# Ai00-X/ai00_server

Hardware: AMD Instinct MI355X
Metric: decode tokens/sec (whole job) (higher is better)
Workload: dtype u8->f16/f32acc; 1 GPU; RWKV-v6-3b int8 decode, batch=32/GPU, greedy, state+tokens resident in HBM; quant=int8, batch_per_gpu=32, parallelism=replicas x1 (no collective)

## Files before the change

ai00_server_amd/build.py:

```python
from __future__ import annotations

import os
import subprocess
import sys

HERE = os.path.dirname(os.path.abspath(__file__))
CSRC = os.path.join(HERE, "csrc")
LIB = os.path.join(HERE, "librwkv_hip.so")
SOURCES = ["rwkv_kernels.hip", "rwkv_engine.cpp", "tokenizer.cpp"]
DEPS = SOURCES + ["rwkv_kernels.h", "gemm_plan.h", "graph_cache.h", "gen_stop.h", "safetensors.hpp", "rwkv_abi.map", os.path.join("..", "..", "include", "rwkv_abi.h"),
               os.path.join("..", "..", "include", "rwkv_runtime.hpp"), os.path.join("..", "..", "include", "rwkv_scheduler.hpp"),
               os.path.join("..", "..", "include", "rwkv_router.hpp"),
               os.path.join("..", "..", "harness", "decode_loop.cpp"), os.path.join("..", "..", "harness", "serve_loop.cpp"),
               os.path.join("..", "..", "harness", "router_loop.cpp")]


def _hipcc() -> str:
    for c in (os.environ.get("HIPCC"), "/opt/rocm/bin/hipcc", "hipcc"):
        if c and (os.path.isabs(c) and os.path.exists(c) or not os.path.isabs(c)):
            return c
    return "hipcc"


STAMP = os.path.join(HERE, ".build_stamp")


def _sources_digest() -> str:
    import hashlib
    h = hashlib.sha256()
    for d in sorted(DEPS):
        with open(os.path.join(CSRC, d), "rb") as f:
            h.update(d.encode())
            h.update(f.read())
# ... 72 lines not shown
```

ai00_server_amd/csrc/gemm_plan.h:

```cpp
#pragma once
#include "rwkv_kernels.h"
#include <algorithm>

namespace rwkv {

struct Opd {
    _Float16 *hi = nullptr, *lo = nullptr;
    int ld = 0;
};

struct ProbSpec {
    const DMat *W = nullptr;
    Opd x;
    int xoff = 0;
    int act = ACT_NONE, post = POST_NONE;
    const float *bias = nullptr, *m0 = nullptr, *m1 = nullptr;
    int ldm = 0;
    float *out = nullptr;
    int ldo = 0;
    bool partial = false;
    Opd oh;
};

struct ProbShape {
    int rows, K, fmt;
    bool partial;
    bool kcopies;
    bool smallk;
};
inline ProbShape shape_of(const ProbSpec &s) {
    return {s.W->rows, s.W->K, s.W->fmt, s.partial, s.post != POST_MIX && s.act == ACT_NONE && !s.bias && !s.oh.hi,
            s.xoff == 0 && s.out && !s.oh.hi && s.post == POST_NONE};
}

inline void fill_prob(GemmProb &g, const ProbSpec &s, long pstride) {
    g.W = s.W->data; g.S = s.W->scales; g.fmt = s.W->fmt; g.rows = s.W->rows; g.K = s.W->K;
    g.xhi = s.x.hi + (s.xoff >> 5) * 512; g.xlo = s.x.lo ? s.x.lo + (s.xoff >> 5) * 512 : nullptr; g.ldx = s.x.ld;
    g.act = s.act; g.post = s.post; g.bias = s.bias; g.m0 = s.m0; g.m1 = s.m1; g.ldm = s.ldm;
    g.out_f32 = s.out; g.ldo = s.ldo; g.partial_stride = pstride;
    g.out_hi = s.oh.hi; g.out_lo = s.oh.lo; g.ldh = s.oh.ld;
}

inline void gemm_variant(int T, bool hilo, int &NT, int &KSW) {
    KSW = 8;
// ... 208 lines not shown
```

ai00_server_amd/csrc/rwkv_engine.cpp:

```cpp
#include <hip/hip_runtime.h>

#include <algorithm>
#include <cmath>
#include <cstdio>
#include <cstdlib>
#include <cstring>
#include <map>
#include <memory>
#include <mutex>
#include <numeric>
#include <optional>
#include <stdexcept>
#include <string>
#include <vector>

#include "../../include/rwkv_abi.h"
#include "gemm_plan.h"
#include "graph_cache.h"
#include "safetensors.hpp"

using namespace rwkv;

static thread_local std::string g_err;
struct RwkvError : std::runtime_error {
// ... 235 lines not shown
    float *d_score_out = nullptr, *h_score_out = nullptr, *d_soft_score = nullptr, *h_soft_score = nullptr;
    Opd opA[6], opM, opY, opK, opO, opL[4];
    long pstride = 0;
    int *d_meta = nullptr, *h_meta = nullptr;
    MetaView dm;
    static constexpr int META_RING = 4;
    hipEvent_t meta_ev[META_RING] = {nullptr, nullptr, nullptr, nullptr};
    int meta_next = 0;
    int *h_tok = nullptr, *dv_tok = nullptr;
    StepPlan last_plan;
    std::vector<size_t> last_ntok;
    std::vector<int> last_opt;
    uint64_t plan_counter = 0, uploaded_id = 0;
    size_t meta_cap = 0;
    int *d_tok_feedback = nullptr, *d_hist = nullptr, *d_amax_i = nullptr;
    int *d_adj_row = nullptr, *d_adj_tok = nullptr;
    float *d_adj_val = nullptr;
    unsigned char *d_allow = nullptr, *h_allow = nullptr;
    int *d_allow_row = nullptr;
    SampStage samp{};
    static constexpr size_t ADJ_CAP = 1 << 16;
    float *d_amax_v = nullptr;
    size_t hist_cap = 0;

    bool profiling = false;
    float prof_ms[RWKV_PROFILE_FAMILIES] = {0};
    int prof_n[RWKV_PROFILE_FAMILIES] = {0};
    hipEvent_t ev0 = nullptr, ev1 = nullptr;

    GraphCacheOf<uint64_t> graphs{64, {}};
    std::optional<GraphCacheOf<int>> greedy_graphs;
    static constexpr int GEN_RING_STEPS = 1024;
    std::vector<GenSlot> gen_host;
    std::vector<char> gen_armed;
    std::vector<std::vector<uint32_t>> gen_prompt;
    std::vector<size_t> gen_ppos;
    std::vector<float *> gen_shadow;
    GenSlot *d_gen = nullptr;
    GenStop *d_gen_stop = nullptr;
    std::vector<char> gen_has_stops;
    unsigned *d_tok_off = nullptr;
    unsigned char *d_tok_bytes = nullptr;
    int n_tok = 0;
    void gen_set_token_bytes(const uint8_t *bytes, const int32_t *lens, size_t n);
    void gen_set_stops(int slot, const rwkv_gen_stops &s);
    size_t gen_stop_tail(int slot, uint8_t *out, size_t cap);
// ... 92 lines not shown
        } else {
            f();
        }
    }
    void prof_collect() {
        HIP_CHECK(hipStreamSynchronize(s_main));
        for (size_t i = 0; i < prof_fam.size(); ++i) {
            float ms = 0;
            HIP_CHECK(hipEventElapsedTime(&ms, prof_ev[2 * i], prof_ev[2 * i + 1]));
            prof_ms[prof_fam[i]] += ms;
            prof_n[prof_fam[i]] += 1;
        }
        prof_fam.clear();
    }

    void load(const rwkv_load_desc &d);
    int gemm(std::vector<ProbSpec> &ps, int T, int fam, const ShiftCommit *commit = nullptr, int cls = CLS_NONE);
    void log_gemm(const std::vector<ProbSpec> &ps, int T, int fam, const char *kind, int variant, int grid, int ksplit, int threads);
    void log_row(const char *kernel, int T, long grid, double bytes);
    int step_max_rows = 0;
    float *lnp_xx_att = nullptr;
    void plan_step(const rwkv_slot_input *in, StepPlan &pl);
    void upload_plan(const StepPlan &pl);
    void run_layers(int T, int n_seq, int n_out, const int *d_token, bool dense);
    void infer(const rwkv_slot_input *in, rwkv_slot_output *out);
    void run_plan(const StepPlan &pl);
    void infer_sample(const rwkv_slot_input *in, const rwkv_sample_params *sp, uint32_t *out_tokens, float *out_probs,
                      uint8_t *emitted, size_t *n_consumed);
    void infer_score(const rwkv_slot_input *in, const uint32_t *const *targets, float *const *out_logp, size_t *n_consumed);
    std::vector<rwkv_slot_input> one_token_each(const std::vector<int> &slots, const uint32_t *tokens) const {
        static const uint32_t none = 0;
        std::vector<rwkv_slot_input> in((size_t)max_batch, rwkv_slot_input{nullptr, 0, RWKV_OPTION_LAST, 0});
        for (size_t i = 0; i < slots.size(); ++i) in[(size_t)slots[i]] = rwkv_slot_input{tokens ? tokens + i : &none, 1, RWKV_OPTION_LAST, 0};
        return in;
    }
};

static bool lora_scope(const std::string &name) {
    if (name.compare(0, 7, "blocks.") != 0) return false;
    size_t i = 7;
    while (i < name.size() && name[i] >= '0' && name[i] <= '9') ++i;
    return i > 7 && i + 1 < name.size() && name[i] == '.';
}

static bool is_quant_target(int version, const std::string &suffix) {
    static const char *att56[] = {"att.receptance.weight", "att.key.weight", "att.value.weight", "att.output.weight", "att.gate.weight"};
    static const char *att7[] = {"att.receptance.weight", "att.key.weight", "att.value.weight", "att.output.weight"};
// ... 370 lines not shown
    for (auto &ev : meta_ev) HIP_CHECK(hipEventCreateWithFlags(&ev, hipEventDisableTiming));
    h_tok = hostalloc<int>((size_t)max_batch, hipHostMallocMapped | hipHostMallocCoherent);
    HIP_CHECK(hipHostGetDevicePointer((void **)&dv_tok, h_tok, 0));
    d_tok_feedback = dalloc<int>(chunk);
    soft_rows_cap = (size_t)std::max(1, max_batch);
    soft_in = dalloc<float>(soft_rows_cap * V);
    soft_out = dalloc<float>(soft_rows_cap * V);
    soft_host = hostalloc<float>(soft_rows_cap * V);
    d_score_tgt = dalloc<unsigned>(chunk); d_score_out = dalloc<float>(chunk);
    h_score_tgt = hostalloc<unsigned>(chunk); h_score_out = hostalloc<float>(chunk);
    d_soft_tgt = dalloc<unsigned>(soft_rows_cap); d_soft_score = dalloc<float>(soft_rows_cap);
    h_soft_tgt = hostalloc<unsigned>(soft_rows_cap); h_soft_score = hostalloc<float>(soft_rows_cap);
    d_adj_row = dalloc<int>(ADJ_CAP); d_adj_tok = dalloc<int>(ADJ_CAP); d_adj_val = dalloc<float>(ADJ_CAP);
    d_allow = dalloc<unsigned char>((size_t)max_batch * V); d_allow_row = dalloc<int>(max_batch);
    h_allow = hostalloc<unsigned char>((size_t)max_batch * V + (size_t)max_batch * 4 + 16);
    const size_t o_adj = (size_t)chunk * sizeof(SampleRow), o_out = o_adj + ADJ_CAP * 12, samp_bytes = o_out + (size_t)chunk * 8;
    unsigned char *h_samp = hostalloc<unsigned char>(samp_bytes);
    unsigned char *dv_samp = nullptr;
    HIP_CHECK(hipHostGetDevicePointer((void **)&dv_samp, h_samp, 0));
    int *adj = (int *)(h_samp + o_adj), *out = (int *)(h_samp + o_out), *dv_out = (int *)(dv_samp + o_out);
    samp = SampStage{(SampleRow *)h_samp, adj, adj + ADJ_CAP, (float *)(adj + 2 * ADJ_CAP), out, (float *)(out + chunk),
                     (const SampleRow *)dv_samp, dv_out, (float *)(dv_out + chunk)};
    greedy_graphs.emplace((size_t)max_batch, GraphExecDeleter{});
    d_amax_v = dalloc<float>((size_t)chunk * 32);
    d_amax_i = dalloc<int>((size_t)chunk * 32);
    HIP_CHECK(hipDeviceSynchronize());
}

int rwkv_engine::gemm(std::vector<ProbSpec> &ps, int T, int fam, const ShiftCommit *commit, int cls) {
    const bool hilo = wide(cls);
    if (hilo) for (auto &sp : ps) if (!sp.x.lo) throw RwkvError(RWKV_ERR_INVALID, "gemm: a hi + lo launch needs the lo part of every operand");
    if (ps.empty() || ps.size() > GEMM_MAXP) throw RwkvError(RWKV_ERR_INVALID, "gemm: bad problem count");
    const int n = (int)ps.size();
    ProbShape sh[GEMM_MAXP];
    for (int i = 0; i < n; ++i) sh[i] = shape_of(ps[i]);
    GemmLaunch Lh;
    const GemmPlan pl = plan_gemm(Lh, sh, n, T, hilo, commit && commit->src, kn);
    if (!pl.ksplit) throw RwkvError(RWKV_ERR_UNSUPPORTED, "cannot split inner dimension");
    for (int i = 0; i < n; ++i) fill_prob(Lh.p[i], ps[i], pstride);
    if (pl.path == GEMM_DECODE && commit) Lh.commit = *commit;
    log_gemm(ps, T, fam, kGemmPathNames[pl.path], pl.variant, pl.grid, pl.ksplit, pl.threads);
    if (pl.path == GEMM_SMALLK) launch(fam, [&] { launch_smallk(Lh, hilo, s_main); });
    else if (pl.path == GEMM_TILE) launch(fam, [&] { launch_gemm_tile(Lh, pl.variant, hilo, s_main); });
    else launch(fam, [&] { launch_gemm(Lh, hilo, s_main); });
    return pl.ksplit;
}

void rwkv_engine::log_row(const char *kernel, int T, long grid, double bytes) {
    if (!launch_log || cur_layer > 1) return;
    std::fprintf(launch_log, "{\"kind\": \"row\", \"kernel\": \"%s\", \"T\": %d, \"grid\": %ld, \"bytes\": %.0f}\n", kernel, T, grid, bytes);
    std::fflush(launch_log);
}
void rwkv_engine::log_gemm(const std::vector<ProbSpec> &ps, int T, int fam, const char *kind, int variant, int grid, int ksplit, int threads) {
    if (!launch_log || (cur_layer > 1 && fam != FAM_HEAD)) return;
    uint64_t bytes = 0;
    double flops = 0;
    long rows = 0;
    std::string names;
    for (auto &sp : ps) {
        bytes += sp.W->bytes;
        rows += sp.W->rows;
        flops += 2.0 * T * (double)sp.W->rows * sp.W->K;
        for (auto &kv : mats)
// ... 71 lines not shown
    last_ntok.assign(B, 0);
    last_opt.assign(B, 0);
    for (int b = 0; b < B; ++b) { last_ntok[b] = in[b].n_tokens; last_opt[b] = in[b].option; }
}

void rwkv_engine::upload_plan(const StepPlan &pl) {
    const int slot = meta_next;
    meta_next = (meta_next + 1) % META_RING;
    HIP_CHECK(hipEventSynchronize(meta_ev[slot]));
    const MetaView h(h_meta + (size_t)slot * meta_cap, chunk, max_batch);
    std::memcpy(h.token, pl.token.data(), pl.T * 4);
    std::memcpy(h.slot, pl.slot.data(), pl.T * 4);
    std::memcpy(h.prev, pl.prev.data(), pl.T * 4);
    std::memcpy(h.last, pl.last.data(), pl.T * 4);
    std::memcpy(h.out_rows, pl.out_rows.data(), pl.n_out * 4);
    std::memcpy(h.seq_slot, pl.seq_slot.data(), pl.n_seq * 4);
    std::memcpy(h.seq_begin, pl.seq_begin.data(), pl.n_seq * 4);
    std::memcpy(h.seq_len, pl.seq_len.data(), pl.n_seq * 4);
    HIP_CHECK(hipMemcpyAsync(d_meta, h.token, meta_cap * 4, hipMemcpyHostToDevice, s_main));
    HIP_CHECK(hipEventRecord(meta_ev[slot], s_main));
    uploaded_id = pl.id;
}

void rwkv_engine::run_layers(int T, int n_seq, int n_out, const int *d_token, bool dense) {
    const int C = info.num_emb, V = info.num_vocab, H = info.num_head, L = info.num_layer;
    const RowMeta rm{d_token, dm.slot, dm.prev, dm.last, dense ? 1 : 0};

    float *cur = xA, *oth = xB;
    int np = 0;
    {
        EmbedArgs e{emb, ln0w, ln0b, d_token, cur, C, V};
        launch(FAM_ROW, [&] { launch_embed(e, T, s_main); });
    }
    for (int l = 0; l < L; ++l) {
        const LayerW &w = layers[l];
        cur_layer = l;
        LnShiftArgs a{};
        a.x_in = cur; a.x_out = oth; a.P = P; a.np = np; a.pstride = pstride;
        a.lnw = w.ln1w; a.lnb = w.ln1b;
        a.sx = sxa + (long)l * C; a.sx_slot_stride = sx_slot_stride;
        a.rm = rm; a.C = C; a.ldh = C;
        std::vector<ProbSpec> ps;
        auto prob = [&](const DMat *W, const Opd &x, int act, float *out, int ldo) {
            ProbSpec s; s.W = W; s.x = x; s.act = act; s.out = out; s.ldo = ldo; return s;
        };
        auto as = [&](const Opd &o, int cls) { Opd r = o; if (!wide(cls)) r.lo = nullptr; return r; };
        const Opd aA[6] = {as(opA[0], CLS_ATT), as(opA[1], CLS_ATT), as(opA[2], CLS_ATT), as(opA[3], CLS_ATT), as(opA[4], CLS_ATT), as(opA[5], CLS_ATT)};
        const Opd aL[4] = {as(opL[0], CLS_LORA2), as(opL[1], CLS_LORA2), as(opL[2], CLS_LORA2), as(opL[3], CLS_LORA2)};
        const Opd aF[2] = {as(opA[0], CLS_FFN1), as(opA[1], CLS_FFN1)};
        const Opd aY = as(opY, CLS_WO), aK = as(opK, CLS_FV), aZ = as(opA[0], CLS_NONE), aM = as(opM, CLS_NONE);
        auto ln_pro = [&](const LnShiftArgs &r, float *xx_pub) {
            LnProArgs lp{};
            lp.x_in = r.x_in; lp.x_out = r.x_out; lp.P = r.P; lp.np = r.np; lp.pstride = r.pstride;
// ... 118 lines not shown
            ProbSpec s = prob(w.Fk, aF[0], ACT_RELU2, nullptr, 0);
            s.oh = aK;
            ps = {s};
            if (info.version != 7) { ProbSpec r = prob(w.Fr, aF[1], ACT_SIGMOID, frr, C); ps.push_back(r); }
            { launch(FAM_ROW, [&] { launch_ln_shift(f, T, s_main); }); log_ln(f); }
            gemm(ps, T, FAM_GEMM, nullptr, CLS_FFN1);
            std::swap(cur, oth);
        }
        {
            ProbSpec s = prob(w.Fv, aK, ACT_NONE, P, C);
            s.partial = true;
            if (info.version != 7) { s.post = POST_MUL; s.m0 = frr; s.ldm = C; }
            ps = {s};
            np = gemm(ps, T, FAM_GEMM, nullptr, CLS_FV);
        }
    }
    if (n_out > 0) {
        Opd aO = opO;
        if (!wide(CLS_HEAD)) aO.lo = nullptr;
        LnOutArgs o{cur, P, np, pstride, lnow, lnob, dense ? nullptr : dm.out_rows, aO.hi, aO.lo, C, C};
        launch(FAM_ROW, [&] { launch_ln_out(o, n_out, s_main); });
        std::vector<ProbSpec> ps(1);
        ps[0].W = head; ps[0].x = aO; ps[0].out = logits; ps[0].ldo = V;
        gemm(ps, n_out, FAM_HEAD, nullptr, CLS_HEAD);
    } else if (np > 0) {
    }
}

void rwkv_engine::run_plan(const StepPlan &pl) {
    if (pl.dense) std::memcpy(h_tok, pl.token.data(), (size_t)pl.T * 4);
    if (!pl.dense || pl.id != uploaded_id) upload_plan(pl);
    const int *tok_ptr = pl.dense ? dv_tok : dm.token;
    step_max_rows = pl.max_rows();
    const bool short_rows = step_max_rows <= 8;
    const uint64_t key = ((uint64_t)pl.dense << 63) | ((uint64_t)short_rows << 62) | ((uint64_t)pl.T << 40) | ((uint64_t)pl.n_seq << 20) | (uint64_t)pl.n_out;
    auto enqueue = [&] { run_layers(pl.T, pl.n_seq, pl.n_out, tok_ptr, pl.dense); };
    if (profiling) return enqueue();
    hipGraphExec_t *exec = graphs.find(key);
    if (!exec) {
        if (!graphs.should_capture(key)) return enqueue();
        exec = &graphs.insert(key, capture(s_main, enqueue));
    }
    HIP_CHECK(hipGraphLaunch(*exec, s_main));
}

void rwkv_engine::infer_sample(const rwkv_slot_input *in, const rwkv_sample_params *sp, uint32_t *out_tokens, float *out_probs,
                               uint8_t *emitted, size_t *n_consumed) {
    HIP_CHECK(hipSetDevice(device));
    if (info.num_vocab > 65536) throw RwkvError(RWKV_ERR_UNSUPPORTED, "on-device sampling needs num_vocab <= 65536");
// ... 826 lines not shown
}

rwkv_status rwkv_decode_greedy(rwkv_engine *e, int32_t n_slots, const uint32_t *first_tokens, int32_t n_steps,
                               uint32_t *out_tokens, float *elapsed_ms) {
    return guard([&] {
        if (!e || !first_tokens || !out_tokens || n_slots <= 0 || n_slots > e->max_batch || n_slots > e->chunk || n_steps <= 0)
            throw RwkvError(RWKV_ERR_INVALID, "bad arguments");
        HIP_CHECK(hipSetDevice(e->device));
        use_knobs(e->kn);
        for (int b = 0; b < n_slots; ++b) e->gen_disarm_slot(b);
        StepPlan pl;
        std::vector<int> slots((size_t)n_slots);
        std::iota(slots.begin(), slots.end(), 0);
        e->plan_step(e->one_token_each(slots, first_tokens).data(), pl);
        e->upload_plan(pl);
        const size_t need = (size_t)n_steps * n_slots;
        if (need > e->hist_cap) {
            if (e->d_hist) {
                e->allocs.erase(std::remove(e->allocs.begin(), e->allocs.end(), (void *)e->d_hist), e->allocs.end());
                (void)hipFree(e->d_hist);
            }
            e->d_hist = e->dalloc<int>(need);
            e->hist_cap = need;
        }
        HIP_CHECK(hipMemcpyAsync(e->d_tok_feedback, first_tokens, n_slots * 4, hipMemcpyHostToDevice, e->s_main));
        HIP_CHECK(hipStreamSynchronize(e->s_main));
        hipGraphExec_t *exec = e->greedy_graphs->find(n_slots);
        if (!exec)
            exec = &e->greedy_graphs->insert(n_slots, capture(e->s_main, [&] {
                e->run_layers(pl.T, pl.n_seq, pl.n_out, e->d_tok_feedback, pl.dense);
                launch_argmax(e->logits, n_slots, e->info.num_vocab, e->d_tok_feedback, e->d_amax_v, e->d_amax_i, e->s_main);
            }));
        HIP_CHECK(hipEventRecord(e->ev0, e->s_main));
        for (int s = 0; s < n_steps; ++s) {
            HIP_CHECK(hipGraphLaunch(*exec, e->s_main));
            HIP_CHECK(hipMemcpyAsync(e->d_hist + (size_t)s * n_slots, e->d_tok_feedback, n_slots * 4, hipMemcpyDeviceToDevice, e->s_main));
        }
        HIP_CHECK(hipEventRecord(e->ev1, e->s_main));
        HIP_CHECK(hipEventSynchronize(e->ev1));
        float ms = 0;
        HIP_CHECK(hipEventElapsedTime(&ms, e->ev0, e->ev1));
        if (elapsed_ms) *elapsed_ms = ms;
        HIP_CHECK(hipMemcpy(out_tokens, e->d_hist, need * 4, hipMemcpyDeviceToHost));
    });
}

rwkv_status rwkv_gen_arm(rwkv_engine *e, int32_t slot, const rwkv_gen_params *p) {
    return guard([&] {
        check_slot(e, slot);
        if (!p) throw RwkvError(RWKV_ERR_INVALID, "null params");
        use_knobs(e->kn);
        e->gen_arm(slot, *p, nullptr, 0);
    });
}
rwkv_status rwkv_gen_arm_prompt(rwkv_engine *e, int32_t slot, const uint32_t *tokens, size_t n_tokens, const rwkv_gen_params *p) {
    return guard([&] {
        check_slot(e, slot);
        if (!p) throw RwkvError(RWKV_ERR_INVALID, "null params");
        if (!tokens || n_tokens == 0) throw RwkvError(RWKV_ERR_INVALID, "a prompt needs at least one token");
// ... 169 lines not shown
```

ai00_server_amd/csrc/rwkv_kernels.h:

```cpp
#pragma once
#ifdef __HIP__
#include <hip/hip_runtime.h>
#else
typedef struct ihipStream_t *hipStream_t;
#ifndef __FLT16_MANT_DIG__
typedef unsigned short _Float16;
#endif
#endif
#include <stddef.h>
#include <stdint.h>

#include "gen_stop.h"

namespace rwkv {

enum WFmt : int { W_F16 = 0, W_INT8 = 1, W_NF4 = 2 };
enum Act : int { ACT_NONE = 0, ACT_TANH = 1, ACT_SIGMOID = 2, ACT_RELU2 = 3, ACT_SILU = 4, ACT_DECAY7 = 5 };
enum Post : int { POST_NONE = 0, POST_MUL = 1, POST_MIX = 2 };

struct Knobs {
    int no_ln_fuse = 0;
    int no_v6_fuse = 0;
    int no_tile = 0, tile_shape = -1;
    int no_dense = 0;
    int tile_ksplit = 1;
    int tile_xcd = -1;
    int promote = -1;
    int v6_ksp_max = 16;
    int v6_ksp_blocks = 160, v6_ksp_min_t = 192;
    static Knobs from_env();
};
const Knobs &knobs();
void use_knobs(const Knobs &k);

constexpr int TILE_ROWS = 16;
constexpr int KSTEP = 32;
constexpr int GEMM_MAX_WAVES = 10;
constexpr int GEMM_MAX_WAVES_K16 = 8;
constexpr int GEMM_MAXP = 8;
constexpr int INT8_BLOCK = 128;
constexpr int NF4_BLOCK = 64;

struct DMat {
    const void *data = nullptr;
    const void *scales = nullptr;
    int fmt = W_F16;
    int rows = 0;
    int K = 0;
    uint64_t bytes = 0;
};

struct RowMeta {
// ... 42 lines not shown
    int block_begin;
    int act, post;
    const float *bias;
    const float *m0, *m1;
    int ldm;
    float *out_f32;
    int ldo;
    long partial_stride;
    _Float16 *out_hi, *out_lo;
    int ldh;
};

struct GemmLaunch {
    GemmProb p[GEMM_MAXP];
    int nprob;
    int T;
    int threads;
    int lds_items;
    int single_shot;
    int tail;
    int total_blocks;
    int xcd_map;
    ShiftCommit commit;
};

size_t lnp_lds_bytes(int T, int C, bool hilo);
void launch_gemm(const GemmLaunch &L, bool hilo, hipStream_t s);
void launch_smallk(const GemmLaunch &L, bool hilo, hipStream_t s);
void launch_gemm_tile45(const GemmLaunch &L, int kind, int ntl, bool hilo, hipStream_t s);
void launch_gemm_tile(const GemmLaunch &L, int shape, bool hilo, hipStream_t s);

struct V6MixArgs {
    const void *W1;
    const void *W2[5];
    const _Float16 *zhi, *zlo;
    int ldz;
    const float *xx, *dx;
    const float *mu[5];
    _Float16 *ohi[5], *olo[5];
    int ldh, T, C, Dm;
    LnProArgs lnp;
    const float *mu_x;
    _Float16 *mg_hi = nullptr, *mg_lo = nullptr;
    float *mp = nullptr;
    int ksp = 1, ksp_min_t = 192, ksp_blocks = 160, ksp_max = 16;
};
// ... 14 lines not shown
    float *sx;
    long sx_slot_stride;
    RowMeta rm;
    int mode;
    int nmix;
    const float *mu[6];
    _Float16 *ohi[6];
    _Float16 *olo[6];
    int ldh;
    float *xx_out, *dx_out;
    int C;
    int xcd_rows = 0;
};
void launch_ln_shift(const LnShiftArgs &a, int T, hipStream_t s);

struct EmbedArgs {
    const _Float16 *emb;
    const float *lnw, *lnb;
    const int *token;
    float *x;
    int C, V;
};
void launch_embed(const EmbedArgs &a, int T, hipStream_t s);

struct LnOutArgs {
    const float *x_in;
    const float *P;
    int np;
    long pstride;
    const float *lnw, *lnb;
    const int *out_rows;
    _Float16 *ohi, *olo;
    int ldh, C;
};
void launch_ln_out(const LnOutArgs &a, int n_out, hipStream_t s);

struct WkvArgs {
    int version;
    int H, C;
    int n_seq;
    const int *seq_slot;
    const int *seq_begin;
    const int *seq_len;
    int dense;
    float *state;
    long slot_stride;
// ... 101 lines not shown
```

ai00_server_amd/csrc/rwkv_kernels.hip:

```cpp
#include "gemm_plan.h"
#include <type_traits>
#include <cstdlib>
#include <algorithm>


#ifdef RWKV_PART
#define RWKV_PART_ON(k) (RWKV_PART == (k))
#else
#define RWKV_PART_ON(k) 1
#endif
#if defined(RWKV_TRACE) && defined(RWKV_PART)
#error "trace builds are single-part"
#endif

namespace rwkv {

typedef _Float16 f16x8 __attribute__((ext_vector_type(8)));
typedef _Float16 f16x4 __attribute__((ext_vector_type(4)));
typedef _Float16 f16x2 __attribute__((ext_vector_type(2)));
typedef float f32x4 __attribute__((ext_vector_type(4)));
typedef float f32x2 __attribute__((ext_vector_type(2)));
typedef unsigned int u32;
typedef unsigned int u32x4 __attribute__((ext_vector_type(4)));
typedef unsigned int u32x2 __attribute__((ext_vector_type(2)));
// ... 371 lines not shown
                    split_hilo(o3, h, l); hh[3] = h; ll[3] = l;
                    const int off = ((((c >> 5) << 2) + ((c >> 3) & 3)) * T + t) * 8 + (c & 7);
                    *(f16x4 *)(op_l + off) = hh;
                    if constexpr (HILO) *(f16x4 *)(op_lo + off) = ll;
                }
            }
        }
    }
    __syncthreads();
}
__device__ __forceinline__ size_t lnp_op_off(int T, int k, int tl) { return (size_t)((k >> 3) * T + tl) * 8; }
#if RWKV_PART_ON(0)
static int knob_env(const char *name, int dflt) {
    const char *v = std::getenv(name);
    return (v && *v) ? std::atoi(v) : dflt;
}
Knobs Knobs::from_env() {
    Knobs k;
    k.no_ln_fuse = knob_env("RWKV_NO_LN_FUSE", 0); k.no_v6_fuse = knob_env("RWKV_NO_V6_FUSE", 0);
    k.no_tile = knob_env("RWKV_NO_TILE", 0); k.tile_shape = knob_env("RWKV_TILE_SHAPE", -1);
    k.no_dense = knob_env("RWKV_NO_DENSE", 0);
    k.tile_ksplit = knob_env("RWKV_TILE_KSPLIT", 1); k.tile_xcd = knob_env("RWKV_TILE_XCD", -1);
    k.promote = knob_env("RWKV_PROMOTE", -1);
    k.v6_ksp_max = knob_env("RWKV_V6_KSP_MAX", 16); k.v6_ksp_blocks = knob_env("RWKV_V6_KSP_BLOCKS", 160); k.v6_ksp_min_t = knob_env("RWKV_V6_KSP_MIN_T", 192);
    return k;
}
static thread_local Knobs t_knobs;
const Knobs &knobs() { return t_knobs; }
void use_knobs(const Knobs &k) { t_knobs = k; }

size_t lnp_lds_bytes(int T, int C, bool hilo) { return (size_t)(2 * T * (C + LNP_PAD) + 64) * 4 + (size_t)T * C * 2 * (hilo ? 2 : 1); }
#endif

__device__ __forceinline__ void shift_commit(const ShiftCommit &c) {
    for (int t = 0; t < c.T; ++t) {
        const int last = c.rm.dense ? t : c.rm.last[t];
        if (last < 0) continue;
        const act_t src = act_buf(c.src);
        float *dst = c.sx + (long)(c.rm.dense ? t : c.rm.slot[t]) * c.sx_slot_stride;
        for (int i = threadIdx.x * 4; i < c.C; i += blockDim.x * 4) *(float4 *)(dst + i) = act_ld4(src, (long)last * c.C + i);
    }
}

#if RWKV_PART_ON(0)
__device__ __forceinline__ int pin_s(int v) { v = __builtin_amdgcn_readfirstlane(v); asm volatile("" : "+s"(v)); return v; }
__device__ __forceinline__ const void *pin_p(const void *p) {
    const unsigned long long v = (unsigned long long)p;
    const unsigned lo = (unsigned)pin_s((int)(unsigned)v), hi = (unsigned)pin_s((int)(unsigned)(v >> 32));
    return (const void *)(((unsigned long long)hi << 32) | lo);
}
template <int NT, int KSW, bool HILO, bool SHOT, bool TAIL, int FMT>
__device__ __forceinline__ void gemm_body(const GemmLaunch &L, const GemmProb &P, unsigned char *smem) {
    constexpr int KW = KSW * 32, SUB = KSW / RS, RK = RS * 32;
    const int tid = threadIdx.x, lane = tid & 63;
    const int wave = __builtin_amdgcn_readfirstlane(tid >> 6);
    const int lb = (int)blockIdx.x - P.block_begin;
    const int kb = P.ksb == 1 ? 0 : lb / P.nblk_strip, sb = lb - kb * P.nblk_strip;
    const int spb = P.spb, nw = P.nw;
    const int strip0 = sb * spb;
    const int nstrip = min(spb, (P.rows >> 4) - strip0);
    const int Kb = P.Kb;
    const int kbeg = kb * Kb, kend = kbeg + Kb;
    const int nslice = P.nslice;
    f32x4 *red = (f32x4 *)smem;

    Nf4Lut lut;
    if constexpr (FMT == W_NF4) lut = make_nf4_lut();

    auto mma_round = [&](const WRound<FMT> &w, f32x4 (&acc)[NT], f32x4 (&acc2)[NT], const f16x8 (&xb)[NT][KSW],
                         const f16x8 (*xl)[HILO ? KSW : 1], int sub, int k0) {
#pragma unroll
        for (int ks = 0; ks < RS; ++ks) {
            if (!TAIL || k0 + (sub * RS + ks) * 32 < kend) {
                const f16x8 a = frag<FMT>(w, ks, lut);
// ... 151 lines not shown
            if (t < L.T) {
                if (e_bias) pb = *(const float4 *)(e_bias + row0);
                if (e_post != POST_NONE) pm0 = act_ld4(bm0, (long)t * e_ldm + row0);
                if (e_post == POST_MIX) pm1 = act_ld4(bm1, (long)t * e_ldm + row0);
            }
        };
        if (wave < nitem) prefetch(wave);
        __syncthreads();
        TRACE_PT(3);
        for (int item = wave; item < nitem; item += nwaves) {
            if (item != wave) prefetch(item);
            const int s = item / NT, nt = item - s * NT;
            const f32x4 *rp = red + ((s * nw) * NT + nt) * 64 + lane;
            f32x4 v4 = rp[0];
            for (int w2 = 1; w2 < nw; w2 += 3) {
                const f32x4 zero = {0.f, 0.f, 0.f, 0.f};
                const f32x4 pa = rp[w2 * NT * 64];
                const f32x4 pb2 = w2 + 1 < nw ? rp[(w2 + 1) * NT * 64] : zero;
                const f32x4 pc = w2 + 2 < nw ? rp[(w2 + 2) * NT * 64] : zero;
                v4 += pa; v4 += pb2; v4 += pc;
            }
            const int row0 = (strip0 + s) * 16 + (lane >> 4) * 4;
            const int t = t0 + nt * 16 + (lane & 15);
            if (t < L.T) {
                float v[4] = {v4[0], v4[1], v4[2], v4[3]};
                if (e_bias) { v[0] += pb.x; v[1] += pb.y; v[2] += pb.z; v[3] += pb.w; }
                apply_act4(e_act, v);
                if (e_post == POST_MUL) {
                    v[0] *= pm0.x; v[1] *= pm0.y; v[2] *= pm0.z; v[3] *= pm0.w;
                } else if (e_post == POST_MIX) {
                    v[0] = pm0.x + pm1.x * v[0]; v[1] = pm0.y + pm1.y * v[1]; v[2] = pm0.z + pm1.z * v[2]; v[3] = pm0.w + pm1.w * v[3];
                }
                if (e_f32) act_st4(bo32, (long)t * e_ldo + row0, make_float4(v[0], v[1], v[2], v[3]));
                if (e_hi) act_store_operand4(boh, bol, e_lo, opd_off(t, row0, e_ldh), make_float4(v[0], v[1], v[2], v[3]));
            }
        }
        if (t0 + NT * 16 < L.T) __syncthreads();
    }
    TRACE_PT(4);
}

template <int NT, int KSW, bool HILO, bool SHOT, bool TAIL>
__global__ __launch_bounds__(((NT == 4 || (NT == 2 && HILO)) ? GEMM_MAX_WAVES_K16 : GEMM_MAX_WAVES) * 64) void gemm_kernel(const GemmLaunch L) {
    extern __shared__ __attribute__((aligned(16))) unsigned char smem[];
    if ((int)blockIdx.x >= L.total_blocks) {
        shift_commit(L.commit);
        return;
    }
    int pi = 0;
    for (int i = 1; i < L.nprob; ++i)
        if ((int)blockIdx.x >= L.p[i].block_begin) pi = i;
    const GemmProb &P = L.p[pi];
    if (P.fmt == W_F16) gemm_body<NT, KSW, HILO, SHOT, TAIL, W_F16>(L, P, smem);
    else if (P.fmt == W_INT8) gemm_body<NT, KSW, HILO, SHOT, false, W_INT8>(L, P, smem);
    else gemm_body<NT, KSW, HILO, SHOT, false, W_NF4>(L, P, smem);
}

void launch_gemm(const GemmLaunch &L, bool hilo, hipStream_t s) {
    int NT, KSW;
    gemm_variant(L.T, hilo, NT, KSW);
    const size_t lds = (size_t)L.lds_items * NT * 64 * 16;
    dim3 grid(L.total_blocks + (L.commit.src ? 1 : 0)), block(L.threads);
    static bool attr_done[16] = {false};
    int dev = 0;
    (void)hipGetDevice(&dev);
#define GEMM_V3(X, sh, tl) X(1, 8, true, sh, tl) X(2, 8, true, sh, tl) X(2, 8, false, sh, tl) X(1, 8, false, sh, tl) X(4, 8, false, sh, tl)
#define GEMM_VARIANTS(X) GEMM_V3(X, true, true) GEMM_V3(X, true, false) GEMM_V3(X, false, true) GEMM_V3(X, false, false)
    if (!attr_done[dev & 15]) {
        const int cap = 160 * 1024;
#define SET_ATTR(a, b, c, d, e) (void)hipFuncSetAttribute((const void *)gemm_kernel<a, b, c, d, e>, hipFuncAttributeMaxDynamicSharedMemorySize, cap);
        GEMM_VARIANTS(SET_ATTR)
#undef SET_ATTR
        attr_done[dev & 15] = true;
    }
    const bool shot = L.single_shot != 0, tail = L.tail != 0;
#define LAUNCH(a, b, c, d, e) if (NT == a && KSW == b && hilo == c && shot == d && tail == e) hipLaunchKernelGGL((gemm_kernel<a, b, c, d, e>), grid, block, lds, s, L);
    GEMM_VARIANTS(LAUNCH)
#undef LAUNCH
#undef GEMM_VARIANTS
#undef GEMM_V3
}

#endif


#if RWKV_PART_ON(1)
template <int NT, bool HILO, int DS, bool LNP, bool WIDE = false, bool P1ONLY = false>
__global__ __launch_bounds__(512) void v6_mix_kernel(const V6MixArgs a) {
    extern __shared__ __attribute__((aligned(16))) unsigned char smem[];
    const int tid = threadIdx.x, lane = tid & 63;
    const int wave = __builtin_amdgcn_readfirstlane(tid >> 6);
    const int c = blockIdx.y;
    const int sg = blockIdx.x;
    const int C = a.C, Dm = a.Dm, T = a.T;
    const int tz = blockIdx.z;
    const int t0 = tz * NT * 16;
    const int KT1 = C >> 5;
    const int ksp = P1ONLY ? a.ksp : 1, kq = P1ONLY ? (int)blockIdx.x : 0;
// ... 1415 lines not shown
}

template <int PT>
__global__ __launch_bounds__(256) void embed_kernel(const EmbedArgs a) {
    constexpr int NTHR = 256;
    __shared__ float red[8];
    const int t = blockIdx.x, C = a.C;
    float4 wv[PT], bv[PT];
    ROW_FOR(i, c) { wv[i] = ld4(a.lnw + c); bv[i] = ld4(a.lnb + c); }
    int tok = a.token[t];
    tok = tok < 0 ? 0 : (tok >= a.V ? a.V - 1 : tok);
    float4 v[PT];
    ROW_FOR(i, c) {
        const f16x4 e = *(const f16x4 *)(a.emb + (long)tok * C + c);
        v[i] = make_float4((float)e[0], (float)e[1], (float)e[2], (float)e[3]);
    }
    row_layernorm<PT>(v, C, wv, bv, red);
    const act_t bx = act_buf(a.x);
    ROW_FOR(i, c) act_st4(bx, (long)t * C + c, v[i]);
}
void launch_embed(const EmbedArgs &a, int T, hipStream_t s) { ROW_DISPATCH(embed_kernel, a.C, T, a); }

template <int PT>
__global__ __launch_bounds__(256) void ln_out_kernel(const LnOutArgs a) {
    constexpr int NTHR = 256;
    __shared__ float red[8];
    const int o = blockIdx.x, C = a.C;
    float4 wv[PT], bv[PT];
    ROW_FOR(i, c) { wv[i] = ld4(a.lnw + c); bv[i] = ld4(a.lnb + c); }
    const int t = a.out_rows ? a.out_rows[o] : o;
    float4 v[PT];
    row_load_sum<PT>(act_buf(a.x_in), act_buf(a.P), a.np, a.pstride, t, C, v);
    row_layernorm<PT>(v, C, wv, bv, red);
    const act_t oh = act_buf(a.ohi), ol = act_buf(a.olo);
    ROW_FOR(i, c) act_store_operand4(oh, ol, a.olo != nullptr, opd_off(o, c, a.ldh), v[i]);
}
void launch_ln_out(const LnOutArgs &a, int n_out, hipStream_t s) { ROW_DISPATCH(ln_out_kernel, a.C, n_out, a); }

__device__ __forceinline__ float sum16(float v) { return row_sum16(v); }
__device__ __forceinline__ float row_sum16x4(float o0, float o1, float o2, float o3, int j) {
    const bool b0 = j & 1, b1 = j & 2;
    const float p0 = (b0 ? o1 : o0) + dpp_f32<0xB1>(b0 ? o0 : o1);
    const float p1 = (b0 ? o3 : o2) + dpp_f32<0xB1>(b0 ? o2 : o3);
    float q = (b1 ? p1 : p0) + dpp_f32<0x4E>(b1 ? p0 : p1);
    q += dpp_f32<0x124>(q);
    q += dpp_f32<0x128>(q);
// ... 1132 lines not shown
```

Baseline: 14130 tokens/s.

## Fuse greedy argmax into head GEMM epilogue and embed next token in one kernel

Adds an AMAX variant of the decode GEMM that reduces each 16-row strip to a per-token partial max and index instead of writing full logits. A new kernel merges the strip partials, writes the chosen token to the feedback and history buffers, and runs the next step's embedding plus layernorm. This removes the logits write and reread, the separate argmax launch, and the per-step device-to-device history copy. In exchange it needs an extra GEMM kernel instantiation set, a device-side history cursor, and it only applies when the head GEMM plans onto the decode path without a K split.

After: 14250 tokens/s, median of 6. No clear change (+0.8%).

```diff
diff --git a/ai00_server_amd/build.py b/ai00_server_amd/build.py
--- a/ai00_server_amd/build.py
+++ b/ai00_server_amd/build.py
@@ -8,7 +8,7 @@
 CSRC = os.path.join(HERE, "csrc")
 LIB = os.path.join(HERE, "librwkv_hip.so")
 SOURCES = ["rwkv_kernels.hip", "rwkv_engine.cpp", "tokenizer.cpp"]
-DEPS = SOURCES + ["rwkv_kernels.h", "gemm_plan.h", "graph_cache.h", "gen_stop.h", "safetensors.hpp", "rwkv_abi.map", os.path.join("..", "..", "include", "rwkv_abi.h"),
+DEPS = SOURCES + ["rwkv_kernels.h", "gemm_plan.h", "graph_cache.h", "gen_stop.h", "greedy_amax.h", "safetensors.hpp", "rwkv_abi.map", os.path.join("..", "..", "include", "rwkv_abi.h"),
                os.path.join("..", "..", "include", "rwkv_runtime.hpp"), os.path.join("..", "..", "include", "rwkv_scheduler.hpp"),
                os.path.join("..", "..", "include", "rwkv_router.hpp"),
                os.path.join("..", "..", "harness", "decode_loop.cpp"), os.path.join("..", "..", "harness", "serve_loop.cpp"),
diff --git a/ai00_server_amd/csrc/gemm_plan.h b/ai00_server_amd/csrc/gemm_plan.h
--- a/ai00_server_amd/csrc/gemm_plan.h
+++ b/ai00_server_amd/csrc/gemm_plan.h
@@ -20,6 +20,8 @@
     int ldo = 0;
     bool partial = false;
     Opd oh;
+    float *amax_v = nullptr;
+    int *amax_i = nullptr;
 };
 
 struct ProbShape {
diff --git a/ai00_server_amd/csrc/greedy_amax.h b/ai00_server_amd/csrc/greedy_amax.h
--- /dev/null
+++ b/ai00_server_amd/csrc/greedy_amax.h
@@ -0,0 +1,23 @@
+#pragma once
+
+#ifndef RWKV_HD
+#ifdef __HIP__
+#define RWKV_HD __host__ __device__
+#else
+#define RWKV_HD
+#endif
+#endif
+
+namespace rwkv {
+
+constexpr int AMAX_NONE = 0x7fffffff;
+RWKV_HD inline float amax_neg_inf() { return -__builtin_huge_valf(); }
+
+RWKV_HD inline void amax_merge(float &best, int &idx, float v, int i) {
+    if (v > best || (v == best && i < idx)) { best = v; idx = i; }
+}
+RWKV_HD inline void amax_take(float &best, int &idx, float v, int i) {
+    amax_merge(best, idx, v, v > amax_neg_inf() ? i : AMAX_NONE);
+}
+
+}
diff --git a/ai00_server_amd/csrc/rwkv_engine.cpp b/ai00_server_amd/csrc/rwkv_engine.cpp
--- a/ai00_server_amd/csrc/rwkv_engine.cpp
+++ b/ai00_server_amd/csrc/rwkv_engine.cpp
@@ -281,6 +281,8 @@
     static constexpr size_t ADJ_CAP = 1 << 16;
     float *d_amax_v = nullptr;
     size_t hist_cap = 0;
+    int **d_hist_cell = nullptr;
+    int *d_greedy_cur = nullptr;
 
     bool profiling = false;
     float prof_ms[RWKV_PROFILE_FAMILIES] = {0};
@@ -419,7 +421,9 @@
     float *lnp_xx_att = nullptr;
     void plan_step(const rwkv_slot_input *in, StepPlan &pl);
     void upload_plan(const StepPlan &pl);
-    void run_layers(int T, int n_seq, int n_out, const int *d_token, bool dense);
+    struct GreedyTail { float *amax_v; int *amax_i; };
+    void run_layers(int T, int n_seq, int n_out, const int *d_token, bool dense, const GreedyTail *tail = nullptr);
+    bool greedy_fused(int n_slots);
     void infer(const rwkv_slot_input *in, rwkv_slot_output *out);
     void run_plan(const StepPlan &pl);
     void infer_sample(const rwkv_slot_input *in, const rwkv_sample_params *sp, uint32_t *out_tokens, float *out_probs,
@@ -836,8 +840,12 @@
     samp = SampStage{(SampleRow *)h_samp, adj, adj + ADJ_CAP, (float *)(adj + 2 * ADJ_CAP), out, (float *)(out + chunk),
                      (const SampleRow *)dv_samp, dv_out, (float *)(dv_out + chunk)};
     greedy_graphs.emplace((size_t)max_batch, GraphExecDeleter{});
-    d_amax_v = dalloc<float>((size_t)chunk * 32);
-    d_amax_i = dalloc<int>((size_t)chunk * 32);
+    const size_t amax_n = (size_t)std::min(max_batch, chunk) * std::max(32, V / 16);
+    d_amax_v = dalloc<float>(amax_n);
+    d_amax_i = dalloc<int>(amax_n);
+    d_hist_cell = dalloc<int *>(1);
+    HIP_CHECK(hipMemset(d_hist_cell, 0, sizeof(int *)));
+    d_greedy_cur = dalloc<int>((size_t)max_batch);
     HIP_CHECK(hipDeviceSynchronize());
 }
 
@@ -853,6 +861,10 @@
     if (!pl.ksplit) throw RwkvError(RWKV_ERR_UNSUPPORTED, "cannot split inner dimension");
     for (int i = 0; i < n; ++i) fill_prob(Lh.p[i], ps[i], pstride);
     if (pl.path == GEMM_DECODE && commit) Lh.commit = *commit;
+    for (int i = 0; i < n; ++i)
+        if (ps[i].amax_v && (n != 1 || pl.path != GEMM_DECODE || Lh.p[i].ksb != 1))
+            throw RwkvError(RWKV_ERR_UNSUPPORTED, "gemm: arg-max partials need a one-problem launch on the decode kernel without a K split");
+    Lh.amax_v = ps[0].amax_v; Lh.amax_i = ps[0].amax_i;
     log_gemm(ps, T, fam, kGemmPathNames[pl.path], pl.variant, pl.grid, pl.ksplit, pl.threads);
     if (pl.path == GEMM_SMALLK) launch(fam, [&] { launch_smallk(Lh, hilo, s_main); });
     else if (pl.path == GEMM_TILE) launch(fam, [&] { launch_gemm_tile(Lh, pl.variant, hilo, s_main); });
@@ -970,13 +982,13 @@
     uploaded_id = pl.id;
 }
 
-void rwkv_engine::run_layers(int T, int n_seq, int n_out, const int *d_token, bool dense) {
+void rwkv_engine::run_layers(int T, int n_seq, int n_out, const int *d_token, bool dense, const GreedyTail *tail) {
     const int C = info.num_emb, V = info.num_vocab, H = info.num_head, L = info.num_layer;
     const RowMeta rm{d_token, dm.slot, dm.prev, dm.last, dense ? 1 : 0};
 
     float *cur = xA, *oth = xB;
     int np = 0;
-    {
+    if (!tail) {
         EmbedArgs e{emb, ln0w, ln0b, d_token, cur, C, V};
         launch(FAM_ROW, [&] { launch_embed(e, T, s_main); });
     }
@@ -1141,9 +1153,19 @@
         launch(FAM_ROW, [&] { launch_ln_out(o, n_out, s_main); });
         std::vector<ProbSpec> ps(1);
         ps[0].W = head; ps[0].x = aO; ps[0].out = logits; ps[0].ldo = V;
+        if (tail) { ps[0].out = nullptr; ps[0].amax_v = tail->amax_v; ps[0].amax_i = tail->amax_i; }
         gemm(ps, n_out, FAM_HEAD, nullptr, CLS_HEAD);
     } else if (np > 0) {
     }
+}
+
+bool rwkv_engine::greedy_fused(int n_slots) {
+    if (kn.no_greedy_fuse) return false;
+    ProbSpec s;
+    s.W = head; s.x = opO; s.out = logits; s.ldo = info.num_vocab;
+    const ProbShape sh = shape_of(s);
+    GemmLaunch Lh;
+    return plan_gemm(Lh, &sh, 1, n_slots, wide(CLS_HEAD), false, kn).path == GEMM_DECODE;
 }
 
 void rwkv_engine::run_plan(const StepPlan &pl) {
@@ -2016,19 +2038,33 @@
             }
             e->d_hist = e->dalloc<int>(need);
             e->hist_cap = need;
-        }
+            HIP_CHECK(hipMemcpy(e->d_hist_cell, &e->d_hist, sizeof(int *), hipMemcpyHostToDevice));
+        }
+        const bool fused = e->greedy_fused(n_slots);
         HIP_CHECK(hipMemcpyAsync(e->d_tok_feedback, first_tokens, n_slots * 4, hipMemcpyHostToDevice, e->s_main));
         HIP_CHECK(hipStreamSynchronize(e->s_main));
+        const EmbedArgs emb0{e->emb, e->ln0w, e->ln0b, e->d_tok_feedback, e->xA, e->info.num_emb, e->info.num_vocab};
+        const rwkv_engine::GreedyTail tail{e->d_amax_v, e->d_amax_i};
         hipGraphExec_t *exec = e->greedy_graphs->find(n_slots);
         if (!exec)
             exec = &e->greedy_graphs->insert(n_slots, capture(e->s_main, [&] {
-                e->run_layers(pl.T, pl.n_seq, pl.n_out, e->d_tok_feedback, pl.dense);
-                launch_argmax(e->logits, n_slots, e->info.num_vocab, e->d_tok_feedback, e->d_amax_v, e->d_amax_i, e->s_main);
+                if (!fused) {
+                    e->run_layers(pl.T, pl.n_seq, pl.n_out, e->d_tok_feedback, pl.dense);
+                    launch_argmax(e->logits, n_slots, e->info.num_vocab, e->d_tok_feedback, e->d_amax_v, e->d_amax_i, e->s_main);
+                    return;
+                }
+                e->run_layers(pl.T, pl.n_seq, pl.n_out, e->d_tok_feedback, pl.dense, &tail);
+                const GreedyFeedArgs f{e->d_amax_v, e->d_amax_i, e->info.num_vocab / 16, e->d_tok_feedback, e->d_hist_cell, e->d_greedy_cur, n_slots, emb0};
+                launch_greedy_feed_embed(f, e->s_main);
             }));
+        if (fused) {
+            HIP_CHECK(hipMemsetAsync(e->d_greedy_cur, 0, (size_t)n_slots * 4, e->s_main));
+            launch_embed(emb0, n_slots, e->s_main);
+        }
         HIP_CHECK(hipEventRecord(e->ev0, e->s_main));
         for (int s = 0; s < n_steps; ++s) {
             HIP_CHECK(hipGraphLaunch(*exec, e->s_main));
-            HIP_CHECK(hipMemcpyAsync(e->d_hist + (size_t)s * n_slots, e->d_tok_feedback, n_slots * 4, hipMemcpyDeviceToDevice, e->s_main));
+            if (!fused) HIP_CHECK(hipMemcpyAsync(e->d_hist + (size_t)s * n_slots, e->d_tok_feedback, n_slots * 4, hipMemcpyDeviceToDevice, e->s_main));
         }
         HIP_CHECK(hipEventRecord(e->ev1, e->s_main));
         HIP_CHECK(hipEventSynchronize(e->ev1));
diff --git a/ai00_server_amd/csrc/rwkv_kernels.h b/ai00_server_amd/csrc/rwkv_kernels.h
--- a/ai00_server_amd/csrc/rwkv_kernels.h
+++ b/ai00_server_amd/csrc/rwkv_kernels.h
@@ -28,6 +28,7 @@
     int promote = -1;
     int v6_ksp_max = 16;
     int v6_ksp_blocks = 160, v6_ksp_min_t = 192;
+    int no_greedy_fuse = 0;
     static Knobs from_env();
 };
 const Knobs &knobs();
@@ -116,6 +117,8 @@
     int total_blocks;
     int xcd_map;
     ShiftCommit commit;
+    float *amax_v;
+    int *amax_i;
 };
 
 size_t lnp_lds_bytes(int T, int C, bool hilo);
@@ -176,6 +179,18 @@
     int C, V;
 };
 void launch_embed(const EmbedArgs &a, int T, hipStream_t s);
+
+struct GreedyFeedArgs {
+    const float *amax_v;
+    const int *amax_i;
+    int nstrip;
+    int *feedback;
+    int *const *hist;
+    int *cursor;
+    int n_slots;
+    EmbedArgs e;
+};
+void launch_greedy_feed_embed(const GreedyFeedArgs &a, hipStream_t s);
 
 struct LnOutArgs {
     const float *x_in;
diff --git a/ai00_server_amd/csrc/rwkv_kernels.hip b/ai00_server_amd/csrc/rwkv_kernels.hip
--- a/ai00_server_amd/csrc/rwkv_kernels.hip
+++ b/ai00_server_amd/csrc/rwkv_kernels.hip
@@ -1,4 +1,5 @@
 #include "gemm_plan.h"
+#include "greedy_amax.h"
 #include <type_traits>
 #include <cstdlib>
 #include <algorithm>
@@ -417,6 +418,7 @@
     k.no_dense = knob_env("RWKV_NO_DENSE", 0);
     k.tile_ksplit = knob_env("RWKV_TILE_KSPLIT", 1); k.tile_xcd = knob_env("RWKV_TILE_XCD", -1);
     k.promote = knob_env("RWKV_PROMOTE", -1);
+    k.no_greedy_fuse = knob_env("RWKV_NO_GREEDY_FUSE", 0);
     k.v6_ksp_max = knob_env("RWKV_V6_KSP_MAX", 16); k.v6_ksp_blocks = knob_env("RWKV_V6_KSP_BLOCKS", 160); k.v6_ksp_min_t = knob_env("RWKV_V6_KSP_MIN_T", 192);
     return k;
 }
@@ -444,7 +446,7 @@
     const unsigned lo = (unsigned)pin_s((int)(unsigned)v), hi = (unsigned)pin_s((int)(unsigned)(v >> 32));
     return (const void *)(((unsigned long long)hi << 32) | lo);
 }
-template <int NT, int KSW, bool HILO, bool SHOT, bool TAIL, int FMT>
+template <int NT, int KSW, bool HILO, bool SHOT, bool TAIL, int FMT, bool AMAX = false>
 __device__ __forceinline__ void gemm_body(const GemmLaunch &L, const GemmProb &P, unsigned char *smem) {
     constexpr int KW = KSW * 32, SUB = KSW / RS, RK = RS * 32;
     const int tid = threadIdx.x, lane = tid & 63;
@@ -642,6 +644,7 @@
             }
             const int row0 = (strip0 + s) * 16 + (lane >> 4) * 4;
             const int t = t0 + nt * 16 + (lane & 15);
+            [[maybe_unused]] float av[4] = {amax_neg_inf(), amax_neg_inf(), amax_neg_inf(), amax_neg_inf()};
             if (t < L.T) {
                 float v[4] = {v4[0], v4[1], v4[2], v4[3]};
                 if (e_bias) { v[0] += pb.x; v[1] += pb.y; v[2] += pb.z; v[3] += pb.w; }
@@ -653,6 +656,34 @@
                 }
                 if (e_f32) act_st4(bo32, (long)t * e_ldo + row0, make_float4(v[0], v[1], v[2], v[3]));
                 if (e_hi) act_store_operand4(boh, bol, e_lo, opd_off(t, row0, e_ldh), make_float4(v[0], v[1], v[2], v[3]));
+                if constexpr (AMAX) { av[0] = v[0]; av[1] = v[1]; av[2] = v[2]; av[3] = v[3]; }
+            }
+            if constexpr (AMAX) {
+                float bv = amax_neg_inf();
+                int bi = AMAX_NONE;
+#pragma unroll
+                for (int j = 0; j < 4; ++j) amax_take(bv, bi, av[j], row0 + j);
+                {
+                    const unsigned uv = __builtin_bit_cast(unsigned, bv), ui = (unsigned)bi;
+                    const auto xv = __builtin_amdgcn_permlane32_swap(uv, uv, false, false);
+                    const auto xi = __builtin_amdgcn_permlane32_swap(ui, ui, false, false);
+                    const unsigned v0 = xv[0], v1 = xv[1], i0 = xi[0], i1 = xi[1];
+                    bv = __builtin_bit_cast(float, v0); bi = (int)i0;
+                    amax_merge(bv, bi, __builtin_bit_cast(float, v1), (int)i1);
+                }
+                {
+                    const unsigned uv = __builtin_bit_cast(unsigned, bv), ui = (unsigned)bi;
+                    const auto xv = __builtin_amdgcn_permlane16_swap(uv, uv, false, false);
+                    const auto xi = __builtin_amdgcn_permlane16_swap(ui, ui, false, false);
+                    const unsigned v0 = xv[0], v1 = xv[1], i0 = xi[0], i1 = xi[1];
+                    bv = __builtin_bit_cast(float, v0); bi = (int)i0;
+                    amax_merge(bv, bi, __builtin_bit_cast(float, v1), (int)i1);
+                }
+                if (lane < 16 && t < L.T) {
+                    const long o = (long)t * (P.rows >> 4) + (strip0 + s);
+                    L.amax_v[o] = bv;
+                    L.amax_i[o] = bi;
+                }
             }
         }
         if (t0 + NT * 16 < L.T) __syncthreads();
@@ -674,6 +705,15 @@
     if (P.fmt == W_F16) gemm_body<NT, KSW, HILO, SHOT, TAIL, W_F16>(L, P, smem);
     else if (P.fmt == W_INT8) gemm_body<NT, KSW, HILO, SHOT, false, W_INT8>(L, P, smem);
     else gemm_body<NT, KSW, HILO, SHOT, false, W_NF4>(L, P, smem);
+}
+
+template <int NT, int KSW, bool HILO, bool SHOT, bool TAIL>
+__global__ __launch_bounds__(((NT == 4 || (NT == 2 && HILO)) ? GEMM_MAX_WAVES_K16 : GEMM_MAX_WAVES) * 64) void gemm_amax_kernel(const GemmLaunch L) {
+    extern __shared__ __attribute__((aligned(16))) unsigned char smem[];
+    const GemmProb &P = L.p[0];
+    if (P.fmt == W_F16) gemm_body<NT, KSW, HILO, SHOT, TAIL, W_F16, true>(L, P, smem);
+    else if (P.fmt == W_INT8) gemm_body<NT, KSW, HILO, SHOT, false, W_INT8, true>(L, P, smem);
+    else gemm_body<NT, KSW, HILO, SHOT, false, W_NF4, true>(L, P, smem);
 }
 
 void launch_gemm(const GemmLaunch &L, bool hilo, hipStream_t s) {
@@ -691,9 +731,18 @@
 #define SET_ATTR(a, b, c, d, e) (void)hipFuncSetAttribute((const void *)gemm_kernel<a, b, c, d, e>, hipFuncAttributeMaxDynamicSharedMemorySize, cap);
         GEMM_VARIANTS(SET_ATTR)
 #undef SET_ATTR
+#define SET_ATTR(a, b, c, d, e) (void)hipFuncSetAttribute((const void *)gemm_amax_kernel<a, b, c, d, e>, hipFuncAttributeMaxDynamicSharedMemorySize, cap);
+        GEMM_VARIANTS(SET_ATTR)
+#undef SET_ATTR
         attr_done[dev & 15] = true;
     }
     const bool shot = L.single_shot != 0, tail = L.tail != 0;
+    if (L.amax_v) {
+#define LAUNCH(a, b, c, d, e) if (NT == a && KSW == b && hilo == c && shot == d && tail == e) hipLaunchKernelGGL((gemm_amax_kernel<a, b, c, d, e>), grid, block, lds, s, L);
+        GEMM_VARIANTS(LAUNCH)
+#undef LAUNCH
+        return;
+    }
 #define LAUNCH(a, b, c, d, e) if (NT == a && KSW == b && hilo == c && shot == d && tail == e) hipLaunchKernelGGL((gemm_kernel<a, b, c, d, e>), grid, block, lds, s, L);
     GEMM_VARIANTS(LAUNCH)
 #undef LAUNCH
@@ -2155,6 +2204,70 @@
 void launch_embed(const EmbedArgs &a, int T, hipStream_t s) { ROW_DISPATCH(embed_kernel, a.C, T, a); }
 
 template <int PT>
+__global__ __launch_bounds__(256) void greedy_feed_embed_kernel(const GreedyFeedArgs a) {
+    constexpr int NTHR = 256;
+    __shared__ float red[8];
+    __shared__ float sh_v[4];
+    __shared__ int sh_i[4];
+    const int t = blockIdx.x, C = a.e.C;
+    float4 wv[PT], bv[PT];
+    ROW_FOR(i, c) { wv[i] = ld4(a.e.lnw + c); bv[i] = ld4(a.e.lnb + c); }
+    float best = amax_neg_inf();
+    int idx = AMAX_NONE;
+    const float *__restrict__ pv = a.amax_v + (long)t * a.nstrip;
+    const int *__restrict__ pi = a.amax_i + (long)t * a.nstrip;
+    if ((a.nstrip & 3) == 0) {
+        for (int s0 = threadIdx.x * 4; s0 < a.nstrip; s0 += NTHR * 16) {
+            float4 lv[4];
+            int4 li[4];
+#pragma unroll
+            for (int j = 0; j < 4; ++j)
+                if (s0 + j * NTHR * 4 < a.nstrip) { lv[j] = *(const float4 *)(pv + s0 + j * NTHR * 4); li[j] = *(const int4 *)(pi + s0 + j * NTHR * 4); }
+#pragma unroll
+            for (int j = 0; j < 4; ++j)
+                if (s0 + j * NTHR * 4 < a.nstrip) {
+                    amax_merge(best, idx, lv[j].x, li[j].x); amax_merge(best, idx, lv[j].y, li[j].y);
+                    amax_merge(best, idx, lv[j].z, li[j].z); amax_merge(best, idx, lv[j].w, li[j].w);
+                }
+        }
+    } else {
+        for (int s0 = threadIdx.x; s0 < a.nstrip; s0 += NTHR * 4) {
+            float lv[4];
+            int li[4];
+#pragma unroll
+            for (int j = 0; j < 4; ++j)
+                if (s0 + j * NTHR < a.nstrip) { lv[j] = pv[s0 + j * NTHR]; li[j] = pi[s0 + j * NTHR]; }
+#pragma unroll
+            for (int j = 0; j < 4; ++j)
+                if (s0 + j * NTHR < a.nstrip) amax_merge(best, idx, lv[j], li[j]);
+        }
+    }
+#pragma unroll
+    for (int k = 32; k >= 1; k >>= 1) amax_merge(best, idx, __shfl_xor(best, k, 64), __shfl_xor(idx, k, 64));
+    if ((threadIdx.x & 63) == 0) { sh_v[threadIdx.x >> 6] = best; sh_i[threadIdx.x >> 6] = idx; }
+    __syncthreads();
+    best = sh_v[0]; idx = sh_i[0];
+#pragma unroll
+    for (int w = 1; w < NTHR / 64; ++w) amax_merge(best, idx, sh_v[w], sh_i[w]);
+    if (threadIdx.x == 0) {
+        a.feedback[t] = idx;
+        const int cur = a.cursor[t];
+        (*a.hist)[(long)cur * a.n_slots + t] = idx;
+        a.cursor[t] = cur + 1;
+    }
+    const int tok = idx < 0 ? 0 : (idx >= a.e.V ? a.e.V - 1 : idx);
+    float4 v[PT];
+    ROW_FOR(i, c) {
+        const f16x4 e = *(const f16x4 *)(a.e.emb + (long)tok * C + c);
+        v[i] = make_float4((float)e[0], (float)e[1], (float)e[2], (float)e[3]);
+    }
+    row_layernorm<PT>(v, C, wv, bv, red);
+    const act_t bx = act_buf(a.e.x);
+    ROW_FOR(i, c) act_st4(bx, (long)t * C + c, v[i]);
+}
+void launch_greedy_feed_embed(const GreedyFeedArgs &a, hipStream_t s) { ROW_DISPATCH(greedy_feed_embed_kernel, a.e.C, a.n_slots, a); }
+
+template <int PT>
 __global__ __launch_bounds__(256) void ln_out_kernel(const LnOutArgs a) {
     constexpr int NTHR = 256;
     __shared__ float red[8];
```
